# IntelLabs/GKL

Measured on AMD Instinct MI355X. Metric: pairhmm_gcups, higher is better.
Workload: dtype f32

## Files before the change

### gkl_amd/csrc/pairhmm_aux_kernels.h

```cpp
#pragma once
#include <hip/hip_runtime.h>
#include <stdint.h>

#include "../../include/gkl_hip_pairhmm.h"
#include "pairhmm_fwd_kernel.h"
#include "pairhmm_multi_sets.h"

namespace gklhip {

struct PrepArgs {
  const uint8_t* hap_bases;
  const int32_t* hap_src;
  const int32_t* hap_len;
  const int32_t* hap_pos;
  const int32_t* hap_group;
  const int32_t* hap_pos_flat;
  uint32_t* stream_flat;
  uint32_t* stream;
  uint8_t* hap_has_n;
  int32_t n_haps;
  int32_t* clear_a; int32_t n_a;
  int32_t* clear_b; int32_t n_b;
  int32_t* clear_c; int32_t n_c;
  const uint4* pull_src; uint4* pull_dst; int32_t pull_n16;
// ... 250 lines not shown

#ifndef GKL_PACK_WINDOW
#define GKL_PACK_WINDOW 96
#endif
constexpr int kPackWindow = GKL_PACK_WINDOW;
constexpr int kJobClasses = 64;
constexpr int kPlanBlock = 1024;

struct PlanArgs {
  FinalizeArgs fa;
  int32_t n_reads, n_haps, n_pairs_i;
  const int64_t* read_off;
  int32_t rpl;
  int32_t max_len;
  int32_t* cnts;
  int32_t* hist;
  int32_t* pos;
  int32_t* order;
  LaneSlot* lanes2;
  const int32_t* hap_orig;
  const int32_t* hap_group;
  const int32_t* hap_pos;
  const int32_t* hap_len;
  FwdJob* jobs;
  FwdJob* sorted;
  const LaneSlot* long_lanes;
  int32_t n_long;
  FwdJob* jobs_long;
  int32_t* long_chunk_jobs;
  int32_t total_cols;
  int32_t wanted_jobs;
  int32_t min_job_cols;
  int32_t packed_by_kernels;
};

__device__ __forceinline__ bool last_block_done(int32_t* arrivals) {
  __shared__ int32_t s_is_last;
  __syncthreads();
  if (threadIdx.x == 0) {
    __threadfence();
    const int32_t before = atomicAdd(arrivals, 1);
    s_is_last = before == (int32_t)gridDim.x - 1 ? 1 : 0;
    __threadfence();
  }
  __syncthreads();
  return s_is_last != 0;
}

__device__ __forceinline__ int32_t ld_cnt(int32_t* p) { return __hip_atomic_load(p, __ATOMIC_RELAXED, __HIP_MEMORY_SCOPE_AGENT); }

__device__ __forceinline__ int job_class(const FwdJob& j, const int32_t* hap_pos, const int32_t* hap_len) {
  const int cols = hap_pos[j.hap_end - 1] + hap_len[j.hap_end - 1] - hap_pos[j.hap_begin];
  const int c = cols >> 7;
  return kJobClasses - 1 - (c < kJobClasses - 1 ? c : kJobClasses - 1);
}

__device__ __forceinline__ void build_jobs_for_chunk(const PlanArgs& a, const LaneSlot* lanes, int c, FwdJob* jobs,
                                                     int32_t* chunk_jobs, int cut_cols, bool by_group, int lane) {
  const LaneSlot sl = lanes[(int64_t)c * kLanes + lane];
  jobs += (int64_t)c * a.n_haps;
  int n_jobs = 0;
  bool prev_need = false;
  uint64_t reads = __ballot(sl.read >= 0 && sl.block == 0);
  for (int k0 = 0; k0 < a.n_haps; k0 += kLanes) {
    const int k = k0 + lane;
    const bool in = k < a.n_haps;
// ... 87 lines not shown
      total += t;
    }
    if (tid == 0) __hip_atomic_store(a.cnts + 4, total, __ATOMIC_RELAXED, __HIP_MEMORY_SCOPE_AGENT);
    int acc = base + inc - sum;
    for (int c = hi; c > lo; c--) { pos[c] = acc; acc += hist[c]; }
  }
  __threadfence();
  __syncthreads();
  GKLHIP_PLAN_STAMP(1);

  for (int r0 = tid; r0 < a.n_reads; r0 += kBatch * kPlanBlock) {
    int f[kBatch];
#pragma unroll
    for (int k = 0; k < kBatch; k++) {
      const int r = r0 + k * kPlanBlock;
      const bool in = r < a.n_reads;
      const int fr = in ? a.fa.read_fail[r] : 0;
      const int64_t len = in ? a.read_off[r + 1] - a.read_off[r] : 0;
      f[k] = (fr > 0 && len <= a.max_len) ? fr : 0;
    }
#pragma unroll
    for (int k = 0; k < kBatch; k++)
      if (f[k] > 0) a.order[atomicAdd(pos + f[k], 1)] = r0 + k * kPlanBlock;
  }
}

__global__ __launch_bounds__(kPlanBlock) void plan_policy_kernel(PlanArgs a) {
  __shared__ int32_t s_i32[kPlanBlock / 64];
  __shared__ int32_t s_wave[kPlanBlock / 64];
  __shared__ int32_t s_hist[2 * kPlanLdsBins];
  const int tid = (int)threadIdx.x, lane = tid & 63, wave = tid >> 6;
  const int nblk = (int)gridDim.x, blk = (int)blockIdx.x;

  {
    int32_t my_fails = 0;
    for (int64_t base = (int64_t)blk * kPlanBlock; base < a.fa.n; base += (int64_t)nblk * kPlanBlock) {
      const int64_t i = base + tid;
      const bool in_range = i < a.fa.n;
      const float v = in_range ? a.fa.raw32[i] : 1.0f;
      const bool fails = in_range && v < 1e-28f;
      const uint64_t mask = __ballot(fails);
      if (mask) {
        const int leader = __builtin_ctzll(mask);
        const int32_t read = fails ? (int32_t)((uint32_t)i / (uint32_t)a.n_haps) : -1;
        const int32_t lead_read = __shfl(read, leader, 64);
        const uint64_t same = __ballot(fails && read == lead_read);
        if (lane == leader) atomicAdd(a.fa.read_fail + lead_read, __builtin_popcountll(same));
        if (fails && read != lead_read) atomicAdd(a.fa.read_fail + read, 1);
        if (lane == 0) my_fails += __builtin_popcountll(mask);
      }
      if (in_range) {
        a.fa.used64[i] = fails ? 1 : 0;
        if (a.fa.mode == kModePacked && !a.packed_by_kernels)
          reinterpret_cast<uint64_t*>(a.fa.out)[i] = fails ? 0ull : (kPackedF32Tag | (uint64_t)__float_as_uint(v));
      }
    }
    if (lane == 0) s_wave[wave] = my_fails;
    __syncthreads();
    if (tid == 0) {
      int total = 0;
      for (int w = 0; w < kPlanBlock / 64; w++) total += s_wave[w];
      if (total) atomicAdd(a.cnts + 0, total);
    }
  }
  if (!last_block_done(a.cnts + 10)) return;
  const int n_fail = ld_cnt(a.cnts + 0);
  if (n_fail == 0) return;
  const uint64_t clk0 = wall_clock64();

  if (a.n_haps + 2 <= kPlanLdsBins) order_affected_reads<true>(a, s_hist, s_hist + kPlanLdsBins, s_i32, tid, clk0);
  else                             order_affected_reads<false>(a, a.hist, a.pos, s_i32, tid, clk0);
  GKLHIP_PLAN_STAMP(2);
}

__global__ __launch_bounds__(kPlanBlock) void plan_pack_kernel(PlanArgs a) {
  const int tid = (int)threadIdx.x, lane = tid & 63, wave = tid >> 6;
  const int nblk = (int)gridDim.x, blk = (int)blockIdx.x;
  if (ld_cnt(a.cnts + 0) == 0) return;
  const uint64_t clk0 = wall_clock64();

  {
    static_assert(kPackWindow <= 2 * kLanes, "the window's lane counts sit in two registers per lane");
    __shared__ int32_t s_pack[kPlanBlock / 64][4][kPackWindow];
    int32_t* s_read = s_pack[wave][0]; int32_t* s_needl = s_pack[wave][1]; int32_t* s_sread = s_pack[wave][2];
    int32_t* s_sneed = s_pack[wave][3];
    const int n = ld_cnt(a.cnts + 4);
    const int n_win = (n + kPackWindow - 1) / kPackWindow;
    for (int w = blk * (kPlanBlock / 64) + wave; w < n_win; w += nblk * (kPlanBlock / 64)) {
      const int w0 = w * kPackWindow;
      const int cnt = min(kPackWindow, n - w0);
      for (int i = lane; i < cnt; i += kLanes) {
        const int r = a.order[w0 + i];
        s_read[i] = r;
        s_needl[i] = (int)((a.read_off[r + 1] - a.read_off[r] + a.rpl) / a.rpl);
      }
      __builtin_amdgcn_wave_barrier();
      if (w == 0 && lane == 0) a.cnts[22] = (int32_t)(wall_clock64() - clk0);
      for (int i = lane; i < cnt; i += kLanes) {
        const int ni = s_needl[i];
        int rank = 0;
// ... 347 lines not shown
```

### gkl_amd/csrc/pairhmm_ctx.h

```cpp
#pragma once

using namespace gklhip;

namespace {
struct EnvSwitches {
  static bool on_unless_zero(const char* name) { const char* v = getenv(name); return !v || atoi(v) != 0; }
  static int integer(const char* name) { const char* v = getenv(name); return v ? atoi(v) : 0; }
  const bool wide_long = on_unless_zero("GKLHIP_WIDE_LONG");
  const bool super_long = on_unless_zero("GKLHIP_SUPER_LONG");
  const bool fused_pairs = on_unless_zero("GKLHIP_FUSED_PAIRS");
  const int64_t fused_max = [] { const char* v = getenv("GKLHIP_FUSED_MAX_PAIRS"); return v ? atoll(v) : -1LL; }();
  const bool xcd_aware = on_unless_zero("GKLHIP_XCD_AWARE");
  const bool timing = getenv("GKLHIP_TIMING") != nullptr;
  const int combine_load = integer("GKL_HIP_COMBINE_LOAD");
  const int target_cols = integer("GKLHIP_TARGET_COLS");
  const int fb_wanted_jobs = integer("GKLHIP_FB_WANTED_JOBS");
  const int plan_blocks = integer("GKLHIP_PLAN_BLOCKS");
  const int finalize_threads = integer("GKL_HIP_FINALIZE_THREADS");
  const int finalize_min = integer("GKL_HIP_FINALIZE_MIN");
  const bool combine = [] { const char* v = getenv("GKL_HIP_COMBINE"); return !(v && v[0] == '0'); }();
  const bool combine_mid = integer("GKL_HIP_COMBINE_MID") != 0;
  const bool quiet = getenv("GKL_HIP_QUIET") != nullptr;
  const bool one_device_engine = integer("GKL_HIP_DEVICE_ENGINES") == 1;
  const int small_read_limit = integer("GKL_HIP_SMALL_READ_LIMIT") == 511 ? 511 : 383;
};
const EnvSwitches g_env;
}

#include "hip_host_common.h"

struct DevCtx {
  gklhip_config cfg;
  int device = 0;
  bool multi_device = false;
  int n_cus = 256;
  int n_xcds = 8;
  int asm_general = 1;
  int speculate_fp64 = 0;
  int small_read_limit = g_env.small_read_limit;
  int mid_combine = g_env.combine_mid ? 1 : 0;
  int lds_oob_zero = 1;
  hipStream_t stream = nullptr;
  DevBuf tab32, tab64;
  DevTables<float> dt32;
  DevTables<double> dt64;
  PinBuf stage_slot[2];
  DevBuf plan_dev_slot[2];
  hipEvent_t stage_free_slot[2] = {nullptr, nullptr};
  hipEvent_t plan_unused_slot[2] = {nullptr, nullptr};
  hipStream_t upload_stream = nullptr;
// ... 30 lines not shown
```

### gkl_amd/csrc/pairhmm_device_pass.h

```cpp
#pragma once

namespace {

int aux_streams(DevCtx* c) {
  if (!c->upload_stream) HIP_TRY(hipStreamCreateWithFlags(&c->upload_stream, hipStreamNonBlocking));
  if (!c->copy_stream) {
    HIP_TRY(hipStreamCreateWithFlags(&c->copy_stream, hipStreamNonBlocking));
    if (!c->pad_stream) HIP_TRY(hipStreamCreateWithFlags(&c->pad_stream, hipStreamNonBlocking));
  }
  return GKLHIP_OK;
}

template <typename T>
int upload_tables(DevCtx* c, const HostTables<T>& h, DevBuf* buf, DevTables<T>* dt) {
  const size_t n = (size_t)kQuals * 2 + kMmEntries;
  int st = buf->reserve(n * sizeof(T));
  if (st) return st;
  T* base = buf->as<T>();
  {
    T* pin = nullptr;
    HIP_TRY(hipHostMalloc(reinterpret_cast<void**>(&pin), n * sizeof(T), hipHostMallocDefault));
    memcpy(pin, h.ph2pr.data(), kQuals * sizeof(T));
    memcpy(pin + kQuals, h.div3.data(), kQuals * sizeof(T));
    memcpy(pin + 2 * kQuals, h.mm.data(), kMmEntries * sizeof(T));
// ... 595 lines not shown
  q.mode = P.finalize_mode;
  q.log10_init_f = host_tables_f32().log10_initial; q.log10_init32_as_f64 = std::log10(std::ldexp(1.0, 120)); q.log10_init_d = host_tables_f64().log10_initial;
  return q;
}
size_t planned_max_jobs(const CallPlan& P) { return (size_t)P.n_reads * (size_t)P.n_haps; }
PlanArgs plan_args(const DevCtx* c, const CallPlan& P, const StagedCall& S) {
  const PlanLayout& L = P.L;
  unsigned char* dp = S.dp;
  const int n_reads = P.n_reads, n_haps = P.n_haps;
  PlanArgs pa;
  pa.fa = finalize_args(c, P, S);
  pa.n_reads = n_reads; pa.n_haps = n_haps; pa.n_pairs_i = (int32_t)P.n_pairs;
  pa.read_off = S.b.read_off;
  pa.rpl = kRplF64Jobs; pa.max_len = kLanes * kRplF64Jobs - 1;
  pa.cnts = c->counters.as<int32_t>();
  pa.hist = c->fail_hist.as<int32_t>();
  pa.pos = pa.hist + (n_haps + 2);
  pa.order = c->fail_order.as<int32_t>();
  pa.lanes2 = c->lanes2.as<LaneSlot>();
  pa.hap_orig = reinterpret_cast<const int32_t*>(dp + L.hap_orig);
  pa.hap_group = reinterpret_cast<const int32_t*>(dp + L.hap_group);
  pa.hap_pos = reinterpret_cast<const int32_t*>(dp + L.hap_pos_flat);
  pa.hap_len = reinterpret_cast<const int32_t*>(dp + L.hap_len);
  pa.jobs = c->jobs.as<FwdJob>();
  pa.sorted = c->jobs.as<FwdJob>() + planned_max_jobs(P);
  pa.long_lanes = reinterpret_cast<const LaneSlot*>(dp + L.long_lanes) + (size_t)P.n_long_main * kLanes;
  pa.n_long = P.n_long64;
  pa.jobs_long = c->jobs_long.as<FwdJob>();
  pa.long_chunk_jobs = c->fail_order.as<int32_t>() + n_reads;
  pa.total_cols = (int32_t)std::min<int64_t>((int64_t)P.hl + n_haps, 0x7fffffff);
  pa.wanted_jobs = g_env.fb_wanted_jobs > 0 ? g_env.fb_wanted_jobs : (int)std::min<int64_t>(kFallbackWantedJobs, std::max<int64_t>(4096, P.n_pairs / 100));
  pa.min_job_cols = 256;
  pa.packed_by_kernels = (P.finalize_mode == kModePacked && !P.per_pair) ? 1 : 0;
  return pa;
}

int launch_prep(DevCtx* c, const CallPlan& P, const StagedCall& S) {
  const bool ev = c->cfg.record_events != 0;
  if (ev) {
    const bool deferred = c->cfg.record_events == 2;
    c->ev = c->ev_ring[deferred ? c->calls % DevCtx::kEventRing : 0];
    c->ring_double[deferred ? c->calls % DevCtx::kEventRing : 0] = P.use_double;
    c->calls++;
    HIP_TRY(hipEventRecord(c->ev[0], S.s));
  }
  const PrepArgs pa = prep_args(c, P, S);
  hipLaunchKernelGGL(prep_kernel, dim3((unsigned)prep_grid(pa, P)), dim3(kPrepBlock), 0, S.s, pa);
  if (P.pull) HIP_TRY(hipEventRecord(c->stage_free_slot[S.slot], S.s));
  return GKLHIP_OK;
}
int reserve_carry(DevCtx* c, const CallPlan& P, StagedCall* S) {
  if (P.n_long_main == 0 && P.n_long64 == 0) return GKLHIP_OK;
  if (int rc = c->carry.reserve(P.striped_carry_bytes + (size_t)super_blocks_max<float>() * 2 * (size_t)P.xsteps * 32)) return rc;
  if (P.xsteps > 0) S->xcarry = c->carry.as<unsigned char>() + P.striped_carry_bytes;
  return GKLHIP_OK;
}
int launch_all_double(DevCtx* c, const CallPlan& P, const StagedCall& S) {
  const bool ev = c->cfg.record_events != 0;
  hipStream_t s = S.s;
  const FwdArgs<double> a = fwd_args<double>(c, P, S);
  if (P.n_main_blocks > 0) launch_stream<double, kRplF64Jobs>(a, P.fma, P.n_main_blocks, s);
  if (P.n_long_main > 0)
    launch_long_jobs<double, kRplF64Wide, kRplF64>(long_main_args(c, P, S, a), P.fma, P.n_long_waves, c->plan.max_read_len, c->carry.as<double>(), P.carry_len, s,
                                                   S.xcarry, P.xsteps, c->counters.as<int32_t>() + 12);
  if (ev) HIP_TRY(hipEventRecord(c->ev[2], s));
  hipLaunchKernelGGL(finalize64_kernel, dim3((unsigned)((P.n_pairs + 255) / 256)), dim3(256), 0, s, finalize_args(c, P, S), 1);
  if (ev) { HIP_TRY(hipEventRecord(c->ev[3], s)); HIP_TRY(hipEventRecord(c->ev[4], s)); }
  HIP_TRY(hipEventRecord(c->policy_done, s));
  return GKLHIP_OK;
}
int launch_main_pass_f32(DevCtx* c, const CallPlan& P, const StagedCall& S, const FwdArgs<float>& a) {
  hipStream_t s = S.s;
  if (P.n_main_blocks > 0 && !P.fused) launch_main_f32(a, P.rpl_main, P.fma, P.n_main_blocks, s);
  if (P.n_long_main > 0) {
    const FwdArgs<float> la = long_main_args(c, P, S, a);
    if (P.rpl_main <= 4) launch_long<float, 4>(la, P.fma, P.n_long_waves, c->carry.as<float>(), P.carry_len, s);
    else                 launch_long_jobs<float, kRplF32, kRplF32>(la, P.fma, P.n_long_waves, c->plan.max_read_len, c->carry.as<float>(), P.carry_len, s, S.xcarry, P.xsteps, c->counters.as<int32_t>() + 12);
  }
  if (c->cfg.record_events != 0) HIP_TRY(hipEventRecord(c->ev[2], s));
  return GKLHIP_OK;
}
int launch_per_pair(DevCtx* c, const CallPlan& P, const StagedCall& S, const FwdArgs<float>& a) {
  const bool ev = c->cfg.record_events != 0;
  hipStream_t s = S.s;
  const FwdArgs<double> d = recompute_args(c, P, S);
  const PairPolicyArgs q = pair_policy_args(c, P, S);
  if (ev) HIP_TRY(hipEventRecord(c->ev[3], s));
  if (P.fused) {
    if (int rc = launch_pair_fused(a, d, q, P.rows, P.fma, P.n_pairs, s, c->speculate_fp64 && g_host_calls_in_flight.load(std::memory_order_relaxed) <= 1)) return rc;
  } else if (P.n_pairs > kTwoStepFrom) {
    if (int rc = c->fail_order.reserve((size_t)P.n_pairs * 4)) return rc;
    if (int rc = launch_pair_policy_two_step(d, q, P.rows, P.fma, P.n_pairs, c->fail_order.as<int32_t>(), s)) return rc;
  } else {
    if (int rc = launch_pair_policy(d, q, P.rows, P.fma, P.n_pairs, s)) return rc;
  }
  if (ev) HIP_TRY(hipEventRecord(c->ev[4], s));
  HIP_TRY(hipEventRecord(c->policy_done, s));
  return GKLHIP_OK;
}
int launch_planned_fp64(DevCtx* c, const CallPlan& P, const StagedCall& S) {
  const bool ev = c->cfg.record_events != 0;
  hipStream_t s = S.s;
  const int n_reads = P.n_reads;
  const int64_t n_pairs = P.n_pairs;
  const size_t max_jobs = planned_max_jobs(P);
  int rc;
  if ((rc = c->fail_order.reserve(((size_t)n_reads + (size_t)P.n_long64) * 4))) return rc;
  if ((rc = c->lanes2.reserve((size_t)n_reads * kLanes * sizeof(LaneSlot)))) return rc;
  if ((rc = c->jobs.reserve(2 * max_jobs * sizeof(FwdJob)))) return rc;
  if (P.n_long64 > 0 && (rc = c->jobs_long.reserve((size_t)P.n_long64 * (size_t)P.n_haps * sizeof(FwdJob)))) return rc;
  const PlanArgs pa = plan_args(c, P, S);
  const int blocks_env = g_env.plan_blocks;
  const int policy_grid = std::max(1, blocks_env > 0 ? blocks_env : (int)std::min<int64_t>(c->n_cus, std::max<int64_t>(16, n_pairs / 4096)));
  const int64_t max_windows = ((int64_t)n_reads + kPackWindow - 1) / kPackWindow;
  const int pack_grid = (int)std::max<int64_t>(1, std::min<int64_t>(kPlanBlocks, (max_windows + kPlanBlock / 64 - 1) / (kPlanBlock / 64)));
  const int jobs_grid = std::max(1, std::min(c->n_cus, blocks_env > 0 ? blocks_env : (int)std::min<int64_t>(kPlanBlocks, std::max<int64_t>(16, n_pairs / 8192))));
  hipLaunchKernelGGL(plan_policy_kernel, dim3((unsigned)policy_grid), dim3(kPlanBlock), 0, s, pa);
  HIP_TRY(hipEventRecord(c->policy_done, s));
  hipLaunchKernelGGL(plan_pack_kernel, dim3((unsigned)pack_grid), dim3(kPlanBlock), 0, s, pa);
  hipLaunchKernelGGL(plan_jobs_kernel, dim3((unsigned)jobs_grid), dim3(kPlanBlock), 0, s, pa);
  const bool side_finalize = finalizes_on_device(P.finalize_mode);
  if (side_finalize) {
    if ((rc = aux_streams(c))) return rc;
    HIP_TRY(hipStreamWaitEvent(c->copy_stream, c->policy_done, 0));
    hipLaunchKernelGGL(finalize32_kernel, dim3((unsigned)((n_pairs + 255) / 256)), dim3(256), 0, c->copy_stream, pa.fa);
    HIP_TRY(hipEventRecord(c->early_copy_done, c->copy_stream));
  }
  FwdArgs<double> d = recompute_args(c, P, S);
  d.chunk_lanes = c->lanes2.as<LaneSlot>();
  d.n_chunks = n_reads;
  d.jobs = c->jobs.as<FwdJob>() + max_jobs;
  if (ev) HIP_TRY(hipEventRecord(c->ev[3], s));
  launch_jobs<double, kRplF64Jobs>(d, P.fma, (int)std::min<int64_t>(n_pairs, (int64_t)c->n_cus * 16), s);
  if (P.n_long64 > 0) {
    int32_t* cnts = c->counters.as<int32_t>();
    FwdArgs<double> ld = d;
    ld.chunk_lanes = pa.long_lanes;
    ld.jobs = c->jobs_long.as<FwdJob>();
    ld.job_count = cnts + 8;
    ld.job_next = cnts + 9;
    launch_long_jobs<double, kRplF64Wide, kRplF64>(ld, P.fma, P.n_long_waves, c->plan.max_read_len, c->carry.as<double>(), P.carry_len, s, S.xcarry, P.xsteps, cnts + 13);
  }
  if (ev) HIP_TRY(hipEventRecord(c->ev[4], s));
  hipLaunchKernelGGL(finalize64_kernel, dim3((unsigned)((n_pairs + 255) / 256)), dim3(256), 0, s, pa.fa, 0);
  if (side_finalize) HIP_TRY(hipStreamWaitEvent(s, c->early_copy_done, 0));
  return GKLHIP_OK;
}
int finish_call(DevCtx* c, const CallPlan& P, const StagedCall& S) {
  const bool ev = c->cfg.record_events != 0;
  hipStream_t s = S.s;
  gklhip_stats& st = c->stats;
// ... 44 lines not shown
  k.kind = small_call_kind(P);
  const bool all_double = k.kind == kSmallDouble || k.kind == kSmallDoubleStream;
  k.f = all_double ? FwdArgs<float>{} : fwd_args<float>(c, P, S);
  k.d = k.kind == kSmallDoubleStream ? fwd_args<double>(c, P, S) : recompute_args(c, P, S);
  k.q = pair_policy_args(c, P, S);
  if (all_double) k.q.raw32 = nullptr;
  k.rpl_main = P.rpl_main; k.main_blocks = P.n_main_blocks; k.rows = P.rows; k.n_pairs = (int32_t)P.n_pairs; k.fma = P.fma;
  k.fused = P.fused ? 1 : 0;
  k.speculate = c->speculate_fp64;
  const bool two_step = k.kind == kSmallTwoStep;
  k.flag_grid = two_step || k.kind == kSmallDoubleStream ? multi_flag_blocks(k.n_pairs) : 0;
  k.recompute_grid = two_step ? multi_recompute_blocks(k.n_pairs) : 0;
  k.list = two_step ? c->fail_order.as<int32_t>() : nullptr;
  memcpy(S.hs + P.L.desc, &k, sizeof k);
  out->desc_pinned = reinterpret_cast<const SmallCall*>(S.hs_dev + P.L.desc);
  out->desc_dev = reinterpret_cast<const SmallCall*>(S.dp + P.L.desc);
  c->last_pairs = P.n_pairs;
  c->last_stream = S.s;
  c->have_last = true;
  c->stats.n_fallback = -1;
}

int launch_call(DevCtx* c, const gklhip_batch* db, const CallPlan& P, double* out_dev, hipStream_t s) {
  if (P.n_pairs == 0) return GKLHIP_OK;
  StagedCall S;
  int rc;
  if ((rc = stage_call(c, db, P, out_dev, s, &S))) return rc;
  if ((rc = launch_prep(c, P, S))) return rc;
  if ((rc = reserve_carry(c, P, &S))) return rc;
  if (c->cfg.record_events != 0) HIP_TRY(hipEventRecord(c->ev[1], s));
  if (P.use_double) {
    rc = launch_all_double(c, P, S);
  } else {
    const FwdArgs<float> a = fwd_args<float>(c, P, S);
    if ((rc = launch_main_pass_f32(c, P, S, a))) return rc;
    rc = P.per_pair ? launch_per_pair(c, P, S, a) : launch_planned_fp64(c, P, S);
  }
  return rc ? rc : finish_call(c, P, S);
}
int run_device(DevCtx* c, const gklhip_batch* db, double* out_dev, int finalize_mode, hipStream_t s, Arrays where) {
  CallPlan P;
  plan_call(c, db, finalize_mode, where, false, call_load(false), &P);
  return launch_call(c, db, P, out_dev, s);
}

}
```

### gkl_amd/csrc/pairhmm_fwd_kernel.h

```cpp
#pragma once
#include <hip/hip_runtime.h>
#include <stdint.h>

#include "pairhmm_pair_forms.h"

namespace gklhip {

constexpr uint32_t kEntIdle = 5u;
constexpr uint32_t kEntSep = 0x80000000u;
constexpr int kLanes = kPairLanes;
typedef const uint32_t __attribute__((address_space(4))) StreamWord;
}
#include "pairhmm_fwd_asm.h"
#ifndef GKLHIP_FAST_ASM
#define GKLHIP_FAST_ASM 1
#endif
namespace gklhip {

template <typename T>
struct DevTables {
  const T* ph2pr;
  const T* div3;
  const T* mm;
};
// ... 10 lines not shown

struct HapGroup {
  int32_t hap_begin, hap_end, stream_begin, pad_;
};

struct LaneSlot {
  int32_t read;
  int32_t block;
};

struct FwdJob {
  int32_t chunk, hap_begin, hap_end;
  int32_t klass;
};

template <typename T>
struct FwdArgs {
  DevBatch b;
  DevTables<T> tab;
  const uint32_t* stream;
  const int32_t* hap_len;
  const int32_t* hap_pos;
  const int32_t* hap_orig;
  const T* y0;
  const uint8_t* hap_has_n;
  const HapGroup* groups;
  int32_t n_groups;
  const LaneSlot* chunk_lanes;
  int32_t n_chunks;
  int32_t chunk_stride;
  T* raw;
  uint64_t* packed_out;
  const uint8_t* packed_only_flagged;
  const FwdJob* jobs;
  const int32_t* job_count;
  int32_t* job_next;
  int32_t asm_general;
  int32_t long_filter;
  int64_t super_steps;
};

constexpr uint64_t kPackedF32Tag = 0xFFFFFFFF00000000ull;
__device__ __forceinline__ uint64_t packed_word(double raw) {
  const uint64_t bits = (uint64_t)__double_as_longlong(raw);
  return (bits & kPackedF32Tag) == kPackedF32Tag ? 0x7FF8000000000000ull : bits;
}

template <typename T>
__device__ __forceinline__ void emit_result(const FwdArgs<T>& a, int64_t idx, T v) {
  a.raw[idx] = v;
  if (a.packed_out) {
    if (sizeof(T) == 4) {
      const float f = (float)v;
      a.packed_out[idx] = f < 1e-28f ? 0ull : (kPackedF32Tag | (uint64_t)__float_as_uint(f));
    } else if (!a.packed_only_flagged || a.packed_only_flagged[idx]) {
      a.packed_out[idx] = packed_word((double)v);
    }
  }
}

__device__ __forceinline__ uint32_t dpp_shr1_keep(uint32_t old, uint32_t src) {
  return (uint32_t)__builtin_amdgcn_update_dpp((int)old, (int)src, 0x138, 0xf, 0xf, false);
}
__device__ __forceinline__ uint32_t dpp_shr1_zero(uint32_t src) {
  return (uint32_t)__builtin_amdgcn_update_dpp(0, (int)src, 0x138, 0xf, 0xf, true);
}
__device__ __forceinline__ uint32_t dpp_shr1_and_nop(uint32_t src, uint32_t mask) {
  uint32_t d;
  asm("s_nop 1\n\tv_and_b32_dpp %0, %1, %2 wave_shr:1 row_mask:0xf bank_mask:0xf bound_ctrl:1" : "=v"(d) : "v"(src), "v"(mask));
  return d;
}
__device__ __forceinline__ float recv_above(float v, uint32_t lmask) {
  return __uint_as_float(dpp_shr1_and_nop(__float_as_uint(v), lmask));
}
__device__ __forceinline__ double recv_above(double v, uint32_t lmask) {
  const uint64_t u = (uint64_t)__double_as_longlong(v);
  const uint32_t lo = dpp_shr1_zero((uint32_t)u) & lmask;
  const uint32_t hi = dpp_shr1_zero((uint32_t)(u >> 32)) & lmask;
  return __longlong_as_double((long long)(((uint64_t)hi << 32) | lo));
}

__device__ __forceinline__ float read_lane(float v, int src) {
  return __uint_as_float((uint32_t)__builtin_amdgcn_readlane((int)__float_as_uint(v), src));
// ... 178 lines not shown

  __device__ __forceinline__ void advance(const T* pr, T* nM, T* nX, T* nY) const {
    nM[0] = mul_prior(m_inner<FMA>(dM, dX, dY, pMM[0], pGAPM[0]), pr[0]);
#pragma unroll
    for (int s = 1; s < RPL; s++)
      nM[s] = mul_prior(m_inner<FMA>(M[s - 1], X[s - 1], Y[s - 1], pMM[s], pGAPM[s]), pr[s]);
#pragma unroll
    for (int s = 0; s < RPL; s++) nY[s] = mul_add2<FMA>(Y[s], pXX[s], M[s], pMY[s]);
    nX[0] = mul_add2<FMA>(rX, pXX[0], rM, pMX[0]);
#pragma unroll
    for (int s = 1; s < RPL; s++) nX[s] = mul_add2<FMA>(nX[s - 1], pXX[s], nM[s - 1], pMX[s]);
  }

  __device__ __forceinline__ void shift_entry(uint32_t entry) {
    uint32_t above;
    asm("s_nop 1\n\tv_and_b32_dpp %0, %1, %2 wave_shr:1 row_mask:0xf bank_mask:0xf bound_ctrl:1"
        : "=v"(above) : "v"(ent), "v"(~direct));
    ent = (entry & direct) | above;
  }

  __device__ __forceinline__ void step_fast(uint32_t entry, int lane) {
    shift_entry(entry);
    T pr[RPL], nM[RPL], nX[RPL], nY[RPL];
    load_priors(ent, lane, pr);
    advance(pr, nM, nX, nY);
#pragma unroll
    for (int s = 0; s < RPL; s++) { M[s] = nM[s]; X[s] = nX[s]; Y[s] = nY[s]; }
    dM = rM; dX = rX; dY = rY;
    fetch_above();
    sM = sM + nM[RPL - 1];
    sX = sX + nX[RPL - 1];
  }

  __device__ __forceinline__ void step_any(const FwdArgs<T>& a, uint32_t entry, int lane,
                                           int hap_begin, int hap_end, int k_cur, int orig_cur, T y0_next) {
    constexpr bool kSelfClearing = sizeof(T) == 4;
    shift_entry(entry);
    const bool sep = (int32_t)ent < 0;
    const bool off = sep || ent == kEntIdle;
    const bool is_n = kCodes == 4 && ent == 4u;
    T pr[RPL], nM[RPL], nX[RPL], nY[RPL];
    load_priors((off || is_n) ? 0u : ent, lane, pr);
    if (kCodes == 4 && __ballot(is_n) != 0) {
      T pn[RPL];
      load_priors_n(lane, pn);
#pragma unroll
      for (int s = 0; s < RPL; s++) pr[s] = is_n ? pn[s] : pr[s];
    }
#pragma unroll
    for (int s = 0; s < RPL; s++) pr[s] = off ? T(0) : pr[s];
    advance(pr, nM, nX, nY);
    const T tM = sM + nM[RPL - 1], tX = sX + nX[RPL - 1];
    T y0n = T(0);
    if (sep) {
      const int k = (int)(ent & 0x7fffffffu);
      if (k == k_cur) {
        if (out_read >= 0) emit_result(a, (int64_t)out_read * a.b.n_haps + orig_cur, sM + sX);
        y0n = y0_next;
      } else {
        const bool mine = (k >= hap_begin) && (k < hap_end);
        if (mine && out_read >= 0) emit_result(a, (int64_t)out_read * a.b.n_haps + a.hap_orig[k], sM + sX);
        if (mine && k + 1 < hap_end) {
          y0n = a.y0[k + 1];
          asm volatile("" :: "v"(y0n));
        }
      }
    }
#pragma unroll
    for (int s = 0; s < RPL; s++) {
      M[s] = (!kSelfClearing && sep) ? T(0) : nM[s];
      X[s] = (!kSelfClearing && sep) ? T(0) : nX[s];
      Y[s] = sep ? ((s == padb_slot) ? y0n : T(0)) : nY[s];
    }
    sM = sep ? T(0) : tM;
    sX = sep ? T(0) : tX;
    dM = rM; dX = rX; dY = rY;
    fetch_above();
  }

  __device__ __forceinline__ void step_win(const FwdArgs<T>& a, uint32_t entry, int lane,
                                           int hap_begin, int hap_end, int k_cur, int orig_cur, T y0_next) {
    shift_entry(entry);
    const bool sep = (int32_t)ent < 0;
    const bool off = sep || ent == kEntIdle;
    const bool is_n = ent == 4u;
    T pr[RPL], nM[RPL], nX[RPL], nY[RPL];
    load_priors((off || is_n) ? 0u : ent, lane, pr);
    if (__ballot(is_n) != 0) {
      asm volatile("" ::: "memory");
      T pn[RPL];
      load_priors_n(lane, pn);
#pragma unroll
      for (int s = 0; s < RPL; s++) pr[s] = is_n ? pn[s] : pr[s];
    }
    advance(pr, nM, nX, nY);
    if (off) {
      asm volatile("" ::: "memory");
#pragma unroll
      for (int s = 0; s < RPL; s++) { nM[s] = T(0); nX[s] = T(0); }
    }
#pragma unroll
    for (int s = 0; s < RPL; s++) { M[s] = nM[s]; X[s] = nX[s]; Y[s] = nY[s]; }
    sM = sM + nM[RPL - 1];
    sX = sX + nX[RPL - 1];
    if (sep) {
      asm volatile("" ::: "memory");
      const int k = (int)(ent & 0x7fffffffu);
      T y0n = T(0);
      if (k == k_cur) {
        if (out_read >= 0) emit_result(a, (int64_t)out_read * a.b.n_haps + orig_cur, sM + sX);
        y0n = y0_next;
      } else {
        const bool mine = (k >= hap_begin) && (k < hap_end);
        if (mine && out_read >= 0) emit_result(a, (int64_t)out_read * a.b.n_haps + a.hap_orig[k], sM + sX);
        if (mine && k + 1 < hap_end) {
          y0n = a.y0[k + 1];
          asm volatile("" :: "v"(y0n));
        }
      }
#pragma unroll
      for (int s = 0; s < RPL; s++) Y[s] = (s == padb_slot) ? y0n : T(0);
      sM = T(0);
      sX = T(0);
    }
    dM = rM; dX = rX; dY = rY;
    fetch_above();
  }

  __device__ __forceinline__ void run(const FwdArgs<T>& a, int lane, int hap_begin, int hap_end) {
    constexpr int U = 8;
    if constexpr (kAsmFast || kAsm64) {
      bool whole = a.asm_general;
      if constexpr (kAsm64) {
        if (whole) {
          if (a.packed_out) whole = false;
          bool any_n = false;
          for (int k = hap_begin + lane; k < hap_end; k += kLanes) any_n |= a.hap_has_n[k] != 0;
          if (__ballot(any_n) != 0) whole = false;
        }
      }
      if (whole) {
        if constexpr (FMA) {
          if constexpr (kAsm64 && RPL == 10)     fwd_asm_run_f64r10(*this, a, lane, hap_begin, hap_end);
          else if constexpr (kAsm64 && RPL == 8) fwd_asm_run_f64r8(*this, a, lane, hap_begin, hap_end);
          else if constexpr (kAsm64 && RPL == 6) fwd_asm_run_f64r6(*this, a, lane, hap_begin, hap_end);
          else if constexpr (kAsm64 && RPL == 4) fwd_asm_run_f64r4(*this, a, lane, hap_begin, hap_end);
          else if constexpr (kAsm64)             fwd_asm_run_f64r2(*this, a, lane, hap_begin, hap_end);
          else if constexpr (RPL == 8)           fwd_asm_run_f32r8(*this, a, lane, hap_begin, hap_end);
          else if constexpr (RPL == 4)           fwd_asm_run_f32r4(*this, a, lane, hap_begin, hap_end);
          else                                   fwd_asm_run_f32r2(*this, a, lane, hap_begin, hap_end);
        } else {
          if constexpr (kAsm64 && RPL == 10)     fwd_asm_run_f64r10n(*this, a, lane, hap_begin, hap_end);
          else if constexpr (kAsm64 && RPL == 8) fwd_asm_run_f64r8n(*this, a, lane, hap_begin, hap_end);
          else if constexpr (kAsm64 && RPL == 6) fwd_asm_run_f64r6n(*this, a, lane, hap_begin, hap_end);
          else if constexpr (kAsm64 && RPL == 4) fwd_asm_run_f64r4n(*this, a, lane, hap_begin, hap_end);
          else if constexpr (kAsm64)             fwd_asm_run_f64r2n(*this, a, lane, hap_begin, hap_end);
          else if constexpr (RPL == 8)           fwd_asm_run_f32r8n(*this, a, lane, hap_begin, hap_end);
          else if constexpr (RPL == 4)           fwd_asm_run_f32r4n(*this, a, lane, hap_begin, hap_end);
          else                                   fwd_asm_run_f32r2n(*this, a, lane, hap_begin, hap_end);
        }
        return;
      }
    }
    const int sb = a.hap_pos[hap_begin];
    StreamWord* sp = (StreamWord*)(a.stream + sb);
    reset_state(a.y0[hap_begin]);
    int t = 0;
    int fast_from = skew_max;
    int k_cur = -1, orig_cur = 0;
    T y0_next = T(0);
    for (int k = hap_begin; k < hap_end; k++) {
      const int sep_at = a.hap_pos[k] - sb + a.hap_len[k];
      if (kCodes == 4 && a.hap_has_n[k]) fast_from = sep_at;
      const int slow_end = fast_from < sep_at ? fast_from : sep_at;
      run_any(a, sp, t, slow_end, lane, hap_begin, hap_end, k_cur, orig_cur, y0_next);
      if constexpr (kAsmFast && RPL == 8 && FMA) {
        fwd_fast_asm_f32r8(*this, sp, t, sep_at, lane);
      } else {
        for (; t + U <= sep_at; t += U) {
          uint32_t e[U];
#pragma unroll
          for (int u = 0; u < U; u++) e[u] = sp[t + u];
#pragma unroll
          for (int u = 0; u < U; u++) step_fast(e[u], lane);
        }
      }
      if (sizeof(T) == 8 && t >= fast_from) {
        if (t + 4 <= sep_at) {
          uint32_t e[4];
#pragma unroll
          for (int u = 0; u < 4; u++) e[u] = sp[t + u];
#pragma unroll
          for (int u = 0; u < 4; u++) step_fast(e[u], lane);
          t += 4;
        }
        for (; t < sep_at; t++) step_fast(sp[t], lane);
      }
      run_any(a, sp, t, sep_at, lane, hap_begin, hap_end, k_cur, orig_cur, y0_next);
      fast_from = sep_at + skew_max + 1;
      k_cur = k;
      orig_cur = a.hap_orig[k];
      y0_next = k + 1 < hap_end ? a.y0[k + 1] : T(0);
    }
    run_any(a, sp, t, fast_from, lane, hap_begin, hap_end, k_cur, orig_cur, y0_next);
  }

  __device__ __forceinline__ void run_any(const FwdArgs<T>& a, StreamWord* sp, int& t, int end,
                                          int lane, int hap_begin, int hap_end, int k_cur, int orig_cur, T y0_next) {
    constexpr int V = 4;
    if (sizeof(T) == 8) {
      for (; t + V <= end; t += V) {
        uint32_t e[V];
#pragma unroll
        for (int u = 0; u < V; u++) e[u] = sp[t + u];
#pragma unroll
        for (int u = 0; u < V; u++) step_win(a, e[u], lane, hap_begin, hap_end, k_cur, orig_cur, y0_next);
      }
      for (; t < end; t++) step_win(a, sp[t], lane, hap_begin, hap_end, k_cur, orig_cur, y0_next);
      return;
    }
    for (; t + V <= end; t += V) {
      uint32_t e[V];
#pragma unroll
      for (int u = 0; u < V; u++) e[u] = sp[t + u];
#pragma unroll
      for (int u = 0; u < V; u++) step_any(a, e[u], lane, hap_begin, hap_end, k_cur, orig_cur, y0_next);
    }
    for (; t < end; t++) step_any(a, sp[t], lane, hap_begin, hap_end, k_cur, orig_cur, y0_next);
  }

  __device__ __forceinline__ void run_stripe(const FwdArgs<T>& a, int lane, int hap_begin, int hap_end,
                                             const T* __restrict__ cin, T* __restrict__ cout, int clen) {
    const int sb = a.hap_pos[hap_begin];
    const uint32_t* __restrict__ sp = a.stream + sb;
    reset_state(a.y0[hap_begin]);
    const int t_end = a.hap_pos[hap_end - 1] - sb + a.hap_len[hap_end - 1] + kLanes;
    T ciM = T(0), ciX = T(0), ciY = T(0), coM = T(0), coX = T(0), coY = T(0);
    if (cout && lane == kLanes - 1) { cout[3 * clen] = M[RPL - 1]; cout[3 * clen + 1] = X[RPL - 1]; cout[3 * clen + 2] = Y[RPL - 1]; }
    if (cin && lane == 0) { dM = cin[3 * clen]; dX = cin[3 * clen + 1]; dY = cin[3 * clen + 2]; }
    for (int t = 0; t < t_end; t++) {
      if (cin) {
        if ((t & 63) == 0) {
          ciM = cin[t + lane]; ciX = cin[clen + t + lane]; ciY = cin[2 * clen + t + lane];
        }
        const T vM = read_lane(ciM, t & 63), vX = read_lane(ciX, t & 63), vY = read_lane(ciY, t & 63);
        if (lane == 0) { rM = vM; rX = vX; rY = vY; }
      }
      step_any(a, sp[t], lane, hap_begin, hap_end, -1, 0, T(0));
      if (cout) {
        const int p = t - (kLanes - 1);
        if (p >= 0) {
          const T bM = read_lane(M[RPL - 1], kLanes - 1), bX = read_lane(X[RPL - 1], kLanes - 1),
                  bY = read_lane(Y[RPL - 1], kLanes - 1);
          if (lane == (p & 63)) { coM = bM; coX = bX; coY = bY; }
          if ((p & 63) == 63 || t == t_end - 1) {
            const int base = p & ~63;
            cout[base + lane] = coM; cout[clen + base + lane] = coX; cout[2 * clen + base + lane] = coY;
          }
        }
      }
    }
  }
};

template <typename T, int RPL, bool FMA>
__device__ __forceinline__ void fwd_stream_block(const FwdArgs<T>& a, int block, unsigned char* lds) {
  using Job = WaveJob<T, RPL, FMA>;
  const int lane = threadIdx.x;
  const int g = block / a.chunk_stride;
  const int chunk = block - g * a.chunk_stride;
  if (chunk >= a.n_chunks) return;
  const HapGroup grp = a.groups[g];
  Job job;
  job.lds = lds;
  job.setup(a, lane, a.chunk_lanes[(int64_t)chunk * kLanes + lane]);
  __syncthreads();
  job.run(a, lane, grp.hap_begin, grp.hap_end);
}
template <typename T, int RPL, bool FMA>
__global__ __launch_bounds__(64) __attribute__((amdgpu_waves_per_eu(sizeof(T) == 8 ? 2 : 4))) void pairhmm_fwd_stream_kernel(FwdArgs<T> a) {
  __shared__ __attribute__((aligned(16))) unsigned char lds[WaveJob<T, RPL, FMA>::kLdsBytes];
  fwd_stream_block<T, RPL, FMA>(a, (int)blockIdx.x, lds);
}

template <typename T, int RPL, bool FMA>
__global__ __launch_bounds__(64) __attribute__((amdgpu_waves_per_eu(sizeof(T) == 8 ? 2 : 4))) void pairhmm_fwd_jobs_kernel(FwdArgs<T> a) {
  using Job = WaveJob<T, RPL, FMA>;
  __shared__ __attribute__((aligned(16))) unsigned char lds[Job::kLdsBytes];
  const int lane = threadIdx.x;
  const int n = *a.job_count;
  Job job;
  job.lds = lds;
  int loaded_chunk = INT32_MIN;
  for (;;) {
    int idx = 0;
    if (lane == 0) idx = atomicAdd(a.job_next, 1);
    idx = __builtin_amdgcn_readfirstlane(idx);
    if (idx >= n) break;
    const FwdJob j = a.jobs[idx];
    if (j.chunk != loaded_chunk) {
      __syncthreads();
      job.setup(a, lane, a.chunk_lanes[(int64_t)j.chunk * kLanes + lane]);
      __syncthreads();
      loaded_chunk = j.chunk;
    }
    job.run(a, lane, j.hap_begin, j.hap_end);
  }
}

struct PairPolicyArgs {
  const float* raw32;
  double* out;
  uint8_t* used64;
  int32_t* count;
  const int32_t* hap_sidx;
// ... 487 lines not shown
```

Measured before the change: 4615.

## Fuse fp32 underflow policy detection into main forward kernel result stores

When the new policy-at-store mode applies (non-fused, non-per-pair, no long reads, RPL 8 fp32), the main forward kernel marks failing results and counts them per read as it writes each result. The plan_policy kernel then runs as a single block that only sums the per-read counts, instead of rescanning every raw result across many blocks. This removes a full pass over the output matrix. In exchange it adds compares and occasional atomics in the main kernel's emit path and relies on asm policy variants fwd_asm_run_f32r8_policy that do not appear in these changes.

Result: no change. 4622, median of 5 (+0.2%).

```diff
diff --git a/gkl_amd/csrc/pairhmm_aux_kernels.h b/gkl_amd/csrc/pairhmm_aux_kernels.h
--- a/gkl_amd/csrc/pairhmm_aux_kernels.h
+++ b/gkl_amd/csrc/pairhmm_aux_kernels.h
@@ -306,6 +306,7 @@
   int32_t wanted_jobs;
   int32_t min_job_cols;
   int32_t packed_by_kernels;
+  int32_t policy_at_store;
 };
 
 __device__ __forceinline__ bool last_block_done(int32_t* arrivals) {
@@ -459,7 +460,17 @@
   const int tid = (int)threadIdx.x, lane = tid & 63, wave = tid >> 6;
   const int nblk = (int)gridDim.x, blk = (int)blockIdx.x;
 
-  {
+  if (a.policy_at_store) {
+    int32_t mine = 0;
+    for (int r = tid; r < a.n_reads; r += kPlanBlock) mine += a.fa.read_fail[r];
+    for (int off = 32; off >= 1; off >>= 1) mine += __shfl_xor(mine, off, 64);
+    if (lane == 0) s_wave[wave] = mine;
+    __syncthreads();
+    int32_t total = 0;
+    for (int w = 0; w < kPlanBlock / 64; w++) total += s_wave[w];
+    if (total == 0) return;
+    if (tid == 0) __hip_atomic_store(a.cnts + 0, total, __ATOMIC_RELAXED, __HIP_MEMORY_SCOPE_AGENT);
+  } else {
     int32_t my_fails = 0;
     for (int64_t base = (int64_t)blk * kPlanBlock; base < a.fa.n; base += (int64_t)nblk * kPlanBlock) {
       const int64_t i = base + tid;
@@ -489,10 +500,9 @@
       for (int w = 0; w < kPlanBlock / 64; w++) total += s_wave[w];
       if (total) atomicAdd(a.cnts + 0, total);
     }
-  }
-  if (!last_block_done(a.cnts + 10)) return;
-  const int n_fail = ld_cnt(a.cnts + 0);
-  if (n_fail == 0) return;
+    if (!last_block_done(a.cnts + 10)) return;
+    if (ld_cnt(a.cnts + 0) == 0) return;
+  }
   const uint64_t clk0 = wall_clock64();
 
   if (a.n_haps + 2 <= kPlanLdsBins) order_affected_reads<true>(a, s_hist, s_hist + kPlanLdsBins, s_i32, tid, clk0);
diff --git a/gkl_amd/csrc/pairhmm_ctx.h b/gkl_amd/csrc/pairhmm_ctx.h
--- a/gkl_amd/csrc/pairhmm_ctx.h
+++ b/gkl_amd/csrc/pairhmm_ctx.h
@@ -16,6 +16,7 @@
   const int target_cols = integer("GKLHIP_TARGET_COLS");
   const int fb_wanted_jobs = integer("GKLHIP_FB_WANTED_JOBS");
   const int plan_blocks = integer("GKLHIP_PLAN_BLOCKS");
+  const bool policy_at_store = on_unless_zero("GKL_HIP_POLICY_AT_STORE");
   const int finalize_threads = integer("GKL_HIP_FINALIZE_THREADS");
   const int finalize_min = integer("GKL_HIP_FINALIZE_MIN");
   const bool combine = [] { const char* v = getenv("GKL_HIP_COMBINE"); return !(v && v[0] == '0'); }();
diff --git a/gkl_amd/csrc/pairhmm_device_pass.h b/gkl_amd/csrc/pairhmm_device_pass.h
--- a/gkl_amd/csrc/pairhmm_device_pass.h
+++ b/gkl_amd/csrc/pairhmm_device_pass.h
@@ -651,6 +651,7 @@
   pa.wanted_jobs = g_env.fb_wanted_jobs > 0 ? g_env.fb_wanted_jobs : (int)std::min<int64_t>(kFallbackWantedJobs, std::max<int64_t>(4096, P.n_pairs / 100));
   pa.min_job_cols = 256;
   pa.packed_by_kernels = (P.finalize_mode == kModePacked && !P.per_pair) ? 1 : 0;
+  pa.policy_at_store = 0;
   return pa;
 }
 
@@ -717,6 +718,9 @@
   HIP_TRY(hipEventRecord(c->policy_done, s));
   return GKLHIP_OK;
 }
+bool policy_at_store(const CallPlan& P) {
+  return g_env.policy_at_store && !P.per_pair && !P.fused && P.n_long_main == 0 && P.rpl_main == kRplF32 && P.n_main_blocks > 0;
+}
 int launch_planned_fp64(DevCtx* c, const CallPlan& P, const StagedCall& S) {
   const bool ev = c->cfg.record_events != 0;
   hipStream_t s = S.s;
@@ -728,14 +732,16 @@
   if ((rc = c->lanes2.reserve((size_t)n_reads * kLanes * sizeof(LaneSlot)))) return rc;
   if ((rc = c->jobs.reserve(2 * max_jobs * sizeof(FwdJob)))) return rc;
   if (P.n_long64 > 0 && (rc = c->jobs_long.reserve((size_t)P.n_long64 * (size_t)P.n_haps * sizeof(FwdJob)))) return rc;
-  const PlanArgs pa = plan_args(c, P, S);
+  PlanArgs pa = plan_args(c, P, S);
+  pa.policy_at_store = policy_at_store(P) ? 1 : 0;
   const int blocks_env = g_env.plan_blocks;
-  const int policy_grid = std::max(1, blocks_env > 0 ? blocks_env : (int)std::min<int64_t>(c->n_cus, std::max<int64_t>(16, n_pairs / 4096)));
+  const int policy_grid = pa.policy_at_store ? 1 : std::max(1, blocks_env > 0 ? blocks_env : (int)std::min<int64_t>(c->n_cus, std::max<int64_t>(16, n_pairs / 4096)));
   const int64_t max_windows = ((int64_t)n_reads + kPackWindow - 1) / kPackWindow;
   const int pack_grid = (int)std::max<int64_t>(1, std::min<int64_t>(kPlanBlocks, (max_windows + kPlanBlock / 64 - 1) / (kPlanBlock / 64)));
   const int jobs_grid = std::max(1, std::min(c->n_cus, blocks_env > 0 ? blocks_env : (int)std::min<int64_t>(kPlanBlocks, std::max<int64_t>(16, n_pairs / 8192))));
+  if (pa.policy_at_store) HIP_TRY(hipEventRecord(c->policy_done, s));
   hipLaunchKernelGGL(plan_policy_kernel, dim3((unsigned)policy_grid), dim3(kPlanBlock), 0, s, pa);
-  HIP_TRY(hipEventRecord(c->policy_done, s));
+  if (!pa.policy_at_store) HIP_TRY(hipEventRecord(c->policy_done, s));
   hipLaunchKernelGGL(plan_pack_kernel, dim3((unsigned)pack_grid), dim3(kPlanBlock), 0, s, pa);
   hipLaunchKernelGGL(plan_jobs_kernel, dim3((unsigned)jobs_grid), dim3(kPlanBlock), 0, s, pa);
   const bool side_finalize = finalizes_on_device(P.finalize_mode);
@@ -846,7 +852,8 @@
   if (P.use_double) {
     rc = launch_all_double(c, P, S);
   } else {
-    const FwdArgs<float> a = fwd_args<float>(c, P, S);
+    FwdArgs<float> a = fwd_args<float>(c, P, S);
+    if (policy_at_store(P)) { a.policy_used64 = c->used64.as<uint8_t>(); a.policy_read_fail = c->read_fail.as<int32_t>(); }
     if ((rc = launch_main_pass_f32(c, P, S, a))) return rc;
     rc = P.per_pair ? launch_per_pair(c, P, S, a) : launch_planned_fp64(c, P, S);
   }
diff --git a/gkl_amd/csrc/pairhmm_fwd_kernel.h b/gkl_amd/csrc/pairhmm_fwd_kernel.h
--- a/gkl_amd/csrc/pairhmm_fwd_kernel.h
+++ b/gkl_amd/csrc/pairhmm_fwd_kernel.h
@@ -66,6 +66,8 @@
   T* raw;
   uint64_t* packed_out;
   const uint8_t* packed_only_flagged;
+  uint8_t* policy_used64;
+  int32_t* policy_read_fail;
   const FwdJob* jobs;
   const int32_t* job_count;
   int32_t* job_next;
@@ -80,9 +82,14 @@
   return (bits & kPackedF32Tag) == kPackedF32Tag ? 0x7FF8000000000000ull : bits;
 }
 
-template <typename T>
-__device__ __forceinline__ void emit_result(const FwdArgs<T>& a, int64_t idx, T v) {
+template <bool kPolicy = false, typename T>
+__device__ __forceinline__ void emit_result(const FwdArgs<T>& a, int32_t read, int64_t idx, T v) {
   a.raw[idx] = v;
+  if (kPolicy && sizeof(T) == 4 && a.policy_used64) {
+    const bool fails = (float)v < 1e-28f;
+    a.policy_used64[idx] = fails ? 1 : 0;
+    if (fails) atomicAdd(a.policy_read_fail + read, 1);
+  }
   if (a.packed_out) {
     if (sizeof(T) == 4) {
       const float f = (float)v;
@@ -327,6 +334,7 @@
     sX = sX + nX[RPL - 1];
   }
 
+  template <bool kPolicy = false>
   __device__ __forceinline__ void step_any(const FwdArgs<T>& a, uint32_t entry, int lane,
                                            int hap_begin, int hap_end, int k_cur, int orig_cur, T y0_next) {
     constexpr bool kSelfClearing = sizeof(T) == 4;
@@ -350,11 +358,11 @@
     if (sep) {
       const int k = (int)(ent & 0x7fffffffu);
       if (k == k_cur) {
-        if (out_read >= 0) emit_result(a, (int64_t)out_read * a.b.n_haps + orig_cur, sM + sX);
+        if (out_read >= 0) emit_result<kPolicy>(a, out_read, (int64_t)out_read * a.b.n_haps + orig_cur, sM + sX);
         y0n = y0_next;
       } else {
         const bool mine = (k >= hap_begin) && (k < hap_end);
-        if (mine && out_read >= 0) emit_result(a, (int64_t)out_read * a.b.n_haps + a.hap_orig[k], sM + sX);
+        if (mine && out_read >= 0) emit_result<kPolicy>(a, out_read, (int64_t)out_read * a.b.n_haps + a.hap_orig[k], sM + sX);
         if (mine && k + 1 < hap_end) {
           y0n = a.y0[k + 1];
           asm volatile("" :: "v"(y0n));
@@ -403,11 +411,11 @@
       const int k = (int)(ent & 0x7fffffffu);
       T y0n = T(0);
       if (k == k_cur) {
-        if (out_read >= 0) emit_result(a, (int64_t)out_read * a.b.n_haps + orig_cur, sM + sX);
+        if (out_read >= 0) emit_result(a, out_read, (int64_t)out_read * a.b.n_haps + orig_cur, sM + sX);
         y0n = y0_next;
       } else {
         const bool mine = (k >= hap_begin) && (k < hap_end);
-        if (mine && out_read >= 0) emit_result(a, (int64_t)out_read * a.b.n_haps + a.hap_orig[k], sM + sX);
+        if (mine && out_read >= 0) emit_result(a, out_read, (int64_t)out_read * a.b.n_haps + a.hap_orig[k], sM + sX);
         if (mine && k + 1 < hap_end) {
           y0n = a.y0[k + 1];
           asm volatile("" :: "v"(y0n));
@@ -422,6 +430,7 @@
     fetch_above();
   }
 
+  template <bool kPolicy = false>
   __device__ __forceinline__ void run(const FwdArgs<T>& a, int lane, int hap_begin, int hap_end) {
     constexpr int U = 8;
     if constexpr (kAsmFast || kAsm64) {
@@ -441,6 +450,7 @@
           else if constexpr (kAsm64 && RPL == 6) fwd_asm_run_f64r6(*this, a, lane, hap_begin, hap_end);
           else if constexpr (kAsm64 && RPL == 4) fwd_asm_run_f64r4(*this, a, lane, hap_begin, hap_end);
           else if constexpr (kAsm64)             fwd_asm_run_f64r2(*this, a, lane, hap_begin, hap_end);
+          else if constexpr (RPL == 8 && kPolicy) fwd_asm_run_f32r8_policy(*this, a, lane, hap_begin, hap_end);
           else if constexpr (RPL == 8)           fwd_asm_run_f32r8(*this, a, lane, hap_begin, hap_end);
           else if constexpr (RPL == 4)           fwd_asm_run_f32r4(*this, a, lane, hap_begin, hap_end);
           else                                   fwd_asm_run_f32r2(*this, a, lane, hap_begin, hap_end);
@@ -450,6 +460,7 @@
           else if constexpr (kAsm64 && RPL == 6) fwd_asm_run_f64r6n(*this, a, lane, hap_begin, hap_end);
           else if constexpr (kAsm64 && RPL == 4) fwd_asm_run_f64r4n(*this, a, lane, hap_begin, hap_end);
           else if constexpr (kAsm64)             fwd_asm_run_f64r2n(*this, a, lane, hap_begin, hap_end);
+          else if constexpr (RPL == 8 && kPolicy) fwd_asm_run_f32r8n_policy(*this, a, lane, hap_begin, hap_end);
           else if constexpr (RPL == 8)           fwd_asm_run_f32r8n(*this, a, lane, hap_begin, hap_end);
           else if constexpr (RPL == 4)           fwd_asm_run_f32r4n(*this, a, lane, hap_begin, hap_end);
           else                                   fwd_asm_run_f32r2n(*this, a, lane, hap_begin, hap_end);
@@ -468,7 +479,7 @@
       const int sep_at = a.hap_pos[k] - sb + a.hap_len[k];
       if (kCodes == 4 && a.hap_has_n[k]) fast_from = sep_at;
       const int slow_end = fast_from < sep_at ? fast_from : sep_at;
-      run_any(a, sp, t, slow_end, lane, hap_begin, hap_end, k_cur, orig_cur, y0_next);
+      run_any<kPolicy>(a, sp, t, slow_end, lane, hap_begin, hap_end, k_cur, orig_cur, y0_next);
       if constexpr (kAsmFast && RPL == 8 && FMA) {
         fwd_fast_asm_f32r8(*this, sp, t, sep_at, lane);
       } else {
@@ -491,15 +502,16 @@
         }
         for (; t < sep_at; t++) step_fast(sp[t], lane);
       }
-      run_any(a, sp, t, sep_at, lane, hap_begin, hap_end, k_cur, orig_cur, y0_next);
+      run_any<kPolicy>(a, sp, t, sep_at, lane, hap_begin, hap_end, k_cur, orig_cur, y0_next);
       fast_from = sep_at + skew_max + 1;
       k_cur = k;
       orig_cur = a.hap_orig[k];
       y0_next = k + 1 < hap_end ? a.y0[k + 1] : T(0);
     }
-    run_any(a, sp, t, fast_from, lane, hap_begin, hap_end, k_cur, orig_cur, y0_next);
-  }
-
+    run_any<kPolicy>(a, sp, t, fast_from, lane, hap_begin, hap_end, k_cur, orig_cur, y0_next);
+  }
+
+  template <bool kPolicy = false>
   __device__ __forceinline__ void run_any(const FwdArgs<T>& a, StreamWord* sp, int& t, int end,
                                           int lane, int hap_begin, int hap_end, int k_cur, int orig_cur, T y0_next) {
     constexpr int V = 4;
@@ -519,9 +531,9 @@
 #pragma unroll
       for (int u = 0; u < V; u++) e[u] = sp[t + u];
 #pragma unroll
-      for (int u = 0; u < V; u++) step_any(a, e[u], lane, hap_begin, hap_end, k_cur, orig_cur, y0_next);
-    }
-    for (; t < end; t++) step_any(a, sp[t], lane, hap_begin, hap_end, k_cur, orig_cur, y0_next);
+      for (int u = 0; u < V; u++) step_any<kPolicy>(a, e[u], lane, hap_begin, hap_end, k_cur, orig_cur, y0_next);
+    }
+    for (; t < end; t++) step_any<kPolicy>(a, sp[t], lane, hap_begin, hap_end, k_cur, orig_cur, y0_next);
   }
 
   __device__ __forceinline__ void run_stripe(const FwdArgs<T>& a, int lane, int hap_begin, int hap_end,
@@ -558,7 +570,7 @@
   }
 };
 
-template <typename T, int RPL, bool FMA>
+template <typename T, int RPL, bool FMA, bool kPolicy = false>
 __device__ __forceinline__ void fwd_stream_block(const FwdArgs<T>& a, int block, unsigned char* lds) {
   using Job = WaveJob<T, RPL, FMA>;
   const int lane = threadIdx.x;
@@ -570,12 +582,12 @@
   job.lds = lds;
   job.setup(a, lane, a.chunk_lanes[(int64_t)chunk * kLanes + lane]);
   __syncthreads();
-  job.run(a, lane, grp.hap_begin, grp.hap_end);
+  job.template run<kPolicy>(a, lane, grp.hap_begin, grp.hap_end);
 }
 template <typename T, int RPL, bool FMA>
 __global__ __launch_bounds__(64) __attribute__((amdgpu_waves_per_eu(sizeof(T) == 8 ? 2 : 4))) void pairhmm_fwd_stream_kernel(FwdArgs<T> a) {
   __shared__ __attribute__((aligned(16))) unsigned char lds[WaveJob<T, RPL, FMA>::kLdsBytes];
-  fwd_stream_block<T, RPL, FMA>(a, (int)blockIdx.x, lds);
+  fwd_stream_block<T, RPL, FMA, sizeof(T) == 4 && RPL == 8>(a, (int)blockIdx.x, lds);
 }
 
 template <typename T, int RPL, bool FMA>
```
